# rajan-dubey8/camouflage-multimodal

Hardware: AMD Instinct MI355X
Metric: images/sec fwd+bwd (fusion model train step: fwd + loss + bwd + clip + AdamW) (higher is better)
Workload: dtype bf16; 1 GPU; BASELINE configs[1] on the path that exists (SURVEY 8d): cross-attention fusion model, packed variable-Nr minibatch (Nr ~ real 303..530 histogram, mean 483), Nk=13 real KG rows, train mode dropout 0.3, random-init weights; batch_per_gpu=16, global_batch=16, rg_dim=128, hidden_dim=256, num_heads=8, parallelism=dp1, precision=bf16 MFMA operands, fp32 accumulate/optimizer

## Files before the change

camouflage_multimodal_amd/csrc/common.h:

```cpp
#pragma once
#include <hip/hip_runtime.h>
#include <stdint.h>

#define CAMO_WAVE 64

enum : uint32_t {
  SITE_ATTN_RG2KG = 1, SITE_ATTN_KG2RG = 2, SITE_FFN_RG = 3, SITE_FFN_KG = 4, SITE_FUSE = 5,
  SITE_HEAD0 = 6,
  SITE_LATE0 = 10
};

struct DropCfg {
  uint32_t seed_lo, seed_hi;
  float p;
  float scale;
  uint32_t thr;
};

__host__ __device__ inline DropCfg make_drop(int training, float p, uint64_t seed) {
  DropCfg d;
  d.seed_lo = (uint32_t)(seed & 0xFFFFFFFFull);
  d.seed_hi = (uint32_t)(seed >> 32);
  d.p = (training && p > 0.f) ? p : 0.f;
  d.scale = d.p > 0.f ? 1.0f / (1.0f - d.p) : 1.0f;
  const double t = (double)d.p * 16777216.0;
  unsigned long long t24 = (unsigned long long)t;
  if ((double)t24 < t) ++t24;
  d.thr = t24 >= 16777216ull ? 0xFFFFFFFFu : (uint32_t)(t24 << 8);
  return d;
}

__device__ __forceinline__ uint32_t fmix32(uint32_t x) {
  x ^= x >> 16; x *= 0x85EBCA6Bu; x ^= x >> 13; x *= 0xC2B2AE35u; x ^= x >> 16;
  return x;
}

__device__ __forceinline__ float drop_mult(const DropCfg& d, uint32_t site, uint32_t idx) {
  const uint32_t x = fmix32((idx + (site * 0x85EBCA77u + d.seed_lo)) ^ d.seed_hi);
  return x >= d.thr ? d.scale : 0.0f;
}

extern "C" __device__ int camo_writelane_i32(int, int, int) __asm("llvm.amdgcn.writelane.i32");
#define SET_LANE(v, s, i) (v) = (uint32_t)camo_writelane_i32((int)(s), (i), (int)(v))

__device__ __forceinline__ float wave_sum(float v) {
#pragma unroll
  for (int o = 32; o > 0; o >>= 1) v += __shfl_xor(v, o, 64);
  return v;
}
template <int CTRL, int ROWMASK>
__device__ __forceinline__ float dpp_add(float v) {
  return v + __int_as_float(__builtin_amdgcn_update_dpp(0, __float_as_int(v), CTRL, ROWMASK, 0xf, true));
}
__device__ __forceinline__ float wave_sum_lane63(float v) {
// ... 35 lines not shown
```

camouflage_multimodal_amd/csrc/fused_rows.hip:

```cpp
#include "fused_rows.h"
#include "shadow_inl.h"
#include "gemm.h"
#include "mfma_inl.h"

namespace {

template <int NT, int KS, bool W_IS_A, int DEPTH, bool USE_ROT = true>
struct Stage {
  static constexpr int TOTAL = NT * KS;
  static constexpr int D = DEPTH < TOTAL ? DEPTH : TOTAL;
  static_assert(!USE_ROT || (KS & (KS - 1)) == 0, "rotated k order: power-of-two k steps");
  u32x4 buf[D];
  const u32x4* wp; int rot;
  __device__ __forceinline__ int keff(int ks) const { return USE_ROT ? ((ks + rot) & (KS - 1)) : ks; }
  __device__ __forceinline__ const u32x4* wptr(int i) const { return wp + 64 * (keff(i / NT) * NT + (i % NT)); }
  __device__ __forceinline__ void prefetch(const u32x4* __restrict__ wp_, int rot_) {
    wp = wp_; rot = rot_;
#pragma unroll
    for (int i = 0; i < D; ++i) buf[i] = *wptr(i);
  }
  __device__ __forceinline__ void run(const char* act, f32x16 (&acc)[NT]) {
    run_f([&](int ks) { return *reinterpret_cast<const bf16x8*>(act + 32 * ks); }, acc);
  }
  template <class F>
  __device__ __forceinline__ void run_f(F&& frag, f32x16 (&acc)[NT]) {
    bf16x8 x = frag(keff(0)), xn = x;
#pragma unroll
    for (int i = 0; i < TOTAL; ++i) {
      const int ks = i / NT, t = i % NT;
      const bf16x8 wf = as_frag(buf[i % D]);
      if (i + D < TOTAL) buf[i % D] = *wptr(i + D);
      if (t == 0) {
        x = xn;
        if (ks + 1 < KS) xn = frag(keff(ks + 1));
      }
      if constexpr (W_IS_A) acc[t] = __builtin_amdgcn_mfma_f32_32x32x16_bf16(wf, x, acc[t], 0, 0, 0);
      else                  acc[t] = __builtin_amdgcn_mfma_f32_32x32x16_bf16(x, wf, acc[t], 0, 0, 0);
      __builtin_amdgcn_sched_barrier(0);
    }
  }
};

__device__ __forceinline__ void stamp(unsigned long long* stamps, int k) {
  if (stamps && threadIdx.x == 0) stamps[(size_t)blockIdx.x * 8 + k] = __builtin_amdgcn_s_memrealtime();
}

template <int LOG2C>
__device__ __forceinline__ void copy_out(const char* lds, int pitch, int col_byte0, us16* dst, int ld, size_t row0, int nrows) {
  for (int c = threadIdx.x; c < (32 << LOG2C); c += 256) {
    const int r = c >> LOG2C, k = c & ((1 << LOG2C) - 1);
    if (r < nrows)
      store16_wt(reinterpret_cast<char*>(dst + (row0 + r) * (size_t)ld) + 16 * k, *reinterpret_cast<const u32x4*>(lds + r * pitch + col_byte0 + 16 * k));
  }
}

__global__ __launch_bounds__(256) void shadow_kernel(const ShadowBatch sb, int total_chunks) {
// ... 84 lines not shown
    for (unsigned i = blockIdx.x * 256 + tid; i < n16; i += gridDim.x * 256) z[i] = u32x4{0u, 0u, 0u, 0u};
  }
  stamp(a.stamps, 3);
}

constexpr int PK = 528;
constexpr int PVC = 192;
constexpr int PT = 260;
constexpr int B_VS = 16 * PK;
template <int OCC> struct BackL;
template <> struct BackL<2> { static constexpr int XH = 0, O = 32 * PT * 4, Y = O + 32 * PR, RED = Y + 32 * PR, LDS = RED + 1024; };
template <> struct BackL<3> { static constexpr int Y = 0, XH = 32 * PR, O = 2 * 32 * PR, RED = O + 32 * PR, LDS = RED + 1024; };
constexpr int B_LDS = BackL<2>::LDS;
static_assert(BackL<3>::O >= 4 * 32 * 192 && BackL<3>::O >= 8448 + 9216 && BackL<2>::O >= 4 * 32 * 192, "attention scratch inside region A");

__device__ __forceinline__ void attn_rg_tile(const BackArgs& a, char* smem, char* bufO, int b, size_t row0, int nrows, int w, int lane) {
  const int tid = threadIdx.x, l31 = lane & 31, h = lane >> 5, Nk = a.Nk;
  char* Ks = smem; char* Vs = smem + B_VS;
  for (int c = tid; c < 16 * 64; c += 256) {
    const int j = c >> 6, ch = c & 63;
    u32x4 v = u32x4{0u, 0u, 0u, 0u};
    if (j < Nk) v = *reinterpret_cast<const u32x4*>(a.KV16 + ((size_t)b * Nk + j) * 512 + 8 * ch);
    if (ch < 32) *reinterpret_cast<u32x4*>(Ks + j * PK + 16 * ch) = v;
    else         *reinterpret_cast<u32x4*>(Vs + j * PV + 16 * (ch - 32)) = v;
  }
  const us16* qrow = a.Q16 + (row0 + min(l31, nrows - 1)) * 256 + 64 * w + 8 * h;
  bf16x8 qf[2][2];
#pragma unroll
  for (int hd = 0; hd < 2; ++hd)
#pragma unroll
    for (int s = 0; s < 2; ++s) qf[hd][s] = as_frag(*reinterpret_cast<const u32x4*>(qrow + 32 * hd + 16 * s));
  __syncthreads();
  const bool dodrop = a.drop.p > 0.f;
  const int q4 = (lane >> 2) & 3, p4 = lane & 3, g1 = (lane >> 4) & 1;
#pragma unroll
  for (int hd = 0; hd < 2; ++hd) {
    const int head = 2 * w + hd;
    f32x16 S = zero16();
#pragma unroll
    for (int s = 0; s < 2; ++s) {
      const bf16x8 kf = *reinterpret_cast<const bf16x8*>(Ks + (l31 & 15) * PK + 2 * (32 * head + 16 * s + 8 * h));
      S = __builtin_amdgcn_mfma_f32_32x32x16_bf16(kf, qf[hd][s], S, 0, 0, 0);
    }
    float e[8];
    rg_softmax(S, h, Nk, e);
    const uint32_t ibase = ((uint32_t)(row0 + l31) * 8u + (uint32_t)head) * (uint32_t)Nk;
    if (dodrop) {
#pragma unroll
      for (int i = 0; i < 8; ++i) e[i] *= drop_mult(a.drop, SITE_ATTN_RG2KG, ibase + (uint32_t)acc_row(i, h));
    }
    const bf16x8 pf = as_frag(u32x4{pack2(e[0], e[1]), pack2(e[2], e[3]), pack2(e[4], e[5]), pack2(e[6], e[7])});
    const char* vp = Vs + (4 * h + q4) * PV + 2 * (32 * head + 16 * g1 + 4 * p4);
    const bf16x8 vf = join(lds_tr16(vp), lds_tr16(vp + 8 * PV));
    const f32x16 O = __builtin_amdgcn_mfma_f32_32x32x16_bf16(vf, pf, zero16(), 0, 0, 0);
#pragma unroll
    for (int g = 0; g < 4; ++g)
      *reinterpret_cast<u32x2*>(bufO + l31 * PR + 2 * (32 * head + 8 * g + 4 * h)) =
          u32x2{pack2(O[4 * g], O[4 * g + 1]), pack2(O[4 * g + 2], O[4 * g + 3])};
  }
}

constexpr int SPLIT_ROWS = 64;
constexpr int PART_FLOATS = 16 + 16 + 16 * 32;
static_assert(PART_FLOATS == FUSED_PART_FLOATS, "fused_rows.h");
// ... 13 lines not shown
#pragma unroll
  for (int c = 0; c < 2; ++c) {
    const us16* p = kbase + (size_t)min(r0 + 32 * c + l31, nr - 1) * 512;
#pragma unroll
    for (int hd = 0; hd < 2; ++hd)
#pragma unroll
      for (int s = 0; s < 2; ++s) kf[c][hd][s] = *reinterpret_cast<const u32x4*>(p + 32 * hd + 16 * s);
  }
#pragma unroll
  for (int c = 0; c < 2; ++c)
#pragma unroll
    for (int i = 0; i < 4; ++i) {
      const int id = lane + 64 * i;
      vv[c][i] = *reinterpret_cast<const u32x4*>(vbase + (size_t)min(r0 + 32 * c + (id >> 3), nr - 1) * 512 + 8 * (id & 7));
    }
  f32x16 S[2][2];
  float mx[2] = {-INFINITY, -INFINITY};
#pragma unroll
  for (int c = 0; c < 2; ++c)
#pragma unroll
    for (int hd = 0; hd < 2; ++hd) {
      S[c][hd] = zero16();
#pragma unroll
      for (int s = 0; s < 2; ++s) S[c][hd] = __builtin_amdgcn_mfma_f32_32x32x16_bf16(as_frag(kf[c][hd][s]), qf[hd][s], S[c][hd], 0, 0, 0);
#pragma unroll
      for (int i = 0; i < 16; ++i) mx[hd] = (r0 + 32 * c + acc_row(i, h) < nr) ? fmaxf(mx[hd], S[c][hd][i]) : mx[hd];
    }
  mx[0] = fmaxf(mx[0], __shfl_xor(mx[0], 32, 64));
  mx[1] = fmaxf(mx[1], __shfl_xor(mx[1], 32, 64));
  stamp(a.stamps, 1);
  f32x16 Z[2] = {zero16(), zero16()};
  float L[2] = {0.f, 0.f};
  const bool dodrop = a.drop.p > 0.f;
  const int q4 = (lane >> 2) & 3, p4 = lane & 3, g1 = (lane >> 4) & 1;
#pragma unroll
  for (int c = 0; c < 2; ++c) {
#pragma unroll
    for (int i = 0; i < 4; ++i) { const int id = lane + 64 * i; *reinterpret_cast<u32x4*>(Vt + (id >> 3) * PVC + 16 * (id & 7)) = vv[c][i]; }
#pragma unroll
    for (int hd = 0; hd < 2; ++hd) {
      float e[16];
#pragma unroll
      for (int i = 0; i < 16; ++i) {
        const int row = r0 + 32 * c + acc_row(i, h);
        e[i] = row < nr ? __expf(S[c][hd][i] - mx[hd]) : 0.f;
        L[hd] += e[i];
        if (dodrop) e[i] *= drop_mult(a.drop, SITE_ATTN_KG2RG, ((uint32_t)(rb + row) * 8u + (uint32_t)(2 * w + hd)) * (uint32_t)Nk + (uint32_t)l31);
      }
#pragma unroll
      for (int s = 0; s < 2; ++s) {
        const bf16x8 ef = as_frag(u32x4{pack2(e[8 * s], e[8 * s + 1]), pack2(e[8 * s + 2], e[8 * s + 3]),
                                        pack2(e[8 * s + 4], e[8 * s + 5]), pack2(e[8 * s + 6], e[8 * s + 7])});
        const char* vp = Vt + (16 * s + 4 * h + q4) * PVC + 2 * (32 * hd + 16 * g1 + 4 * p4);
        const bf16x8 vf = join(lds_tr16(vp), lds_tr16(vp + 8 * PVC));
        Z[hd] = __builtin_amdgcn_mfma_f32_32x32x16_bf16(ef, vf, Z[hd], 0, 0, 0);
      }
    }
  }
  L[0] += __shfl_xor(L[0], 32, 64);
  L[1] += __shfl_xor(L[1], 32, 64);
  stamp(a.stamps, 2);
#pragma unroll
// ... 4 lines not shown
      __hip_atomic_store(part + 16 + lane, L[hd], __ATOMIC_RELAXED, __HIP_MEMORY_SCOPE_AGENT);
    }
    float* zt = reinterpret_cast<float*>(Vt);
#pragma unroll
    for (int i = 0; i < 8; ++i) zt[acc_row(i, h) * 32 + l31] = Z[hd][i];
#pragma unroll
    for (int r = 0; r < 2; ++r) {
      const int idx = lane + 64 * r;
      const f32x4 v = *reinterpret_cast<const f32x4*>(zt + 4 * idx);
      float* dst = part + 32 + 4 * idx;
      asm volatile("global_store_dwordx4 %0, %1, off sc1\n\ts_nop 1" ::"v"(dst), "v"(v) : "memory");
    }
  }
}

__device__ __forceinline__ void attn_kg_combine(const BackArgs& a, char* smem, char* bufO, int b, int nsplit) {
  const int tid = threadIdx.x, Nk = a.Nk;
  float* sc = reinterpret_cast<float*>(smem);
  float* invL = sc + nsplit * 128;
  const float* part = a.part + (size_t)a.tile_off[b] * 8 * PART_FLOATS;
  constexpr size_t SS = (size_t)2 * 8 * PART_FLOATS;
  f32x4 zv[4][4];
  auto load_z = [&](int s0) {
#pragma unroll
    for (int k = 0; k < 4; ++k) {
      const float* z = part + (size_t)min(s0 + k, nsplit - 1) * SS + 32;
#pragma unroll
      for (int it = 0; it < 4; ++it) {
        const int idx = tid + 256 * it;
        zv[k][it] = *reinterpret_cast<const f32x4*>(z + (size_t)(idx >> 7) * PART_FLOATS + 4 * (idx & 127));
      }
    }
  };
  load_z(0);
  if (tid < 128) {
    const int hd = tid >> 4, j = tid & 15;
    const float* p0 = part + (size_t)hd * PART_FLOATS + j;
    float M = -INFINITY, L = 0.f;
    if (nsplit <= 16) {
      float mv[16], lv[16];
#pragma unroll
      for (int k = 0; k < 16; ++k) { const size_t o = (size_t)min(k, nsplit - 1) * SS; mv[k] = p0[o]; lv[k] = p0[o + 16]; }
#pragma unroll
      for (int k = 0; k < 16; ++k) M = fmaxf(M, mv[k]);
#pragma unroll
      for (int k = 0; k < 16; ++k)
        if (k < nsplit) { const float e = __expf(mv[k] - M); sc[k * 128 + tid] = e; L = fmaf(lv[k], e, L); }
    } else {
      for (int s0 = 0; s0 < nsplit; s0 += 8) {
        float mv[8];
#pragma unroll
        for (int k = 0; k < 8; ++k) mv[k] = p0[(size_t)min(s0 + k, nsplit - 1) * SS];
#pragma unroll
        for (int k = 0; k < 8; ++k) M = fmaxf(M, mv[k]);
      }
      for (int s0 = 0; s0 < nsplit; s0 += 8) {
        float mv[8], lv[8];
#pragma unroll
        for (int k = 0; k < 8; ++k) { const size_t o = (size_t)min(s0 + k, nsplit - 1) * SS; mv[k] = p0[o]; lv[k] = p0[o + 16]; }
#pragma unroll
        for (int k = 0; k < 8; ++k)
          if (s0 + k < nsplit) { const float e = __expf(mv[k] - M); sc[(s0 + k) * 128 + tid] = e; L = fmaf(lv[k], e, L); }
      }
    }
    invL[tid] = 1.0f / L;
    if ((a.save | a.save_lse2) && a.lse2 && j < Nk) { float* o = a.lse2 + (((size_t)b * 8 + hd) * 16 + j) * 2; o[0] = M; o[1] = L; }
  }
  __syncthreads();
  f32x4 acc[4];
#pragma unroll
  for (int it = 0; it < 4; ++it) acc[it] = f32x4{0.f, 0.f, 0.f, 0.f};
  for (int s0 = 0; s0 < nsplit; s0 += 4) {
    if (s0 > 0) load_z(s0);
#pragma unroll
    for (int k = 0; k < 4; ++k)
      if (s0 + k < nsplit) {
#pragma unroll
        for (int it = 0; it < 4; ++it) acc[it] += zv[k][it] * sc[(s0 + k) * 128 + ((tid + 256 * it) >> 3)];
      }
  }
#pragma unroll
// ... 14 lines not shown
  const int w = __builtin_amdgcn_readfirstlane(tid >> 6);
  const int nkg = a.B * a.max_splits;
  const int vid = (int)blockIdx.x < a.lead_tiles ? nkg + (int)blockIdx.x : ((int)blockIdx.x < a.lead_tiles + nkg ? (int)blockIdx.x - a.lead_tiles : (int)blockIdx.x);
  const bool kg = vid < nkg;
  int rot = ROT ? (int)(blockIdx.x >> 3) : 0;
  using L = BackL<OCC>;
  char* bufO = smem + L::O; char* bufY = smem + L::Y;
  float* red = reinterpret_cast<float*>(smem + L::RED);
  float* tile32 = reinterpret_cast<float*>(smem);
  int b; size_t rowg0; int nrows; float inv_n;
  stamp(a.stamps, 0);
  const BackStream& S = a.s[kg ? 1 : 0];
  Stage<2, 16, true, DEPTH> sto;
  Stage<4, 16, false, DEPTH> stf;
  if (!kg) sto.prefetch(reinterpret_cast<const u32x4*>(S.Wo) + (size_t)w * (16 * 2 * 64) + lane, rot);
  if (kg) {
    b = vid / a.max_splits;
    const int sp = vid - b * a.max_splits;
    if (ROT) rot = b;
    const int nsplit = (a.off[b + 1] - a.off[b] + SPLIT_ROWS - 1) / SPLIT_ROWS;
    if (sp >= nsplit) return;
    attn_kg_split(a, smem, b, sp, w, lane);
    stamp(a.stamps, 4);
    asm volatile("s_waitcnt vmcnt(0)" ::: "memory");
    __syncthreads();
    int* flag = reinterpret_cast<int*>(red);
    if (tid == 0) flag[0] = __hip_atomic_fetch_add(a.tickets + b, 1, __ATOMIC_RELAXED, __HIP_MEMORY_SCOPE_AGENT);
    __syncthreads();
    stamp(a.stamps, 5);
    if (flag[0] != nsplit - 1) return;
    if (tid == 0) {
      __builtin_amdgcn_fence(__ATOMIC_ACQUIRE, "agent");
      asm volatile("s_waitcnt vmcnt(0)" ::: "memory");
    }
    for (int c = tid; c < 32 * PR / 16; c += 256) reinterpret_cast<u32x4*>(bufO)[c] = u32x4{0u, 0u, 0u, 0u};
    __syncthreads();
    sto.prefetch(reinterpret_cast<const u32x4*>(S.Wo) + (size_t)w * (16 * 2 * 64) + lane, rot);
    attn_kg_combine(a, smem, bufO, b, nsplit);
    stamp(a.stamps, 6);
    rowg0 = (size_t)b * a.Nk; nrows = a.Nk; inv_n = 1.0f / (float)a.Nk;
  } else {
    const int4 td = a.tile_desc[vid - nkg];
    if (td.x < 0) return;
    b = td.x; rowg0 = td.y; nrows = td.z; inv_n = __int_as_float(td.w);
    attn_rg_tile(a, smem, bufO, b, rowg0, nrows, w, lane);
  }
  __syncthreads();
  stamp(a.stamps, 1);

  const size_t rrow = rowg0 + min(l31, nrows - 1);
  float u[32];
  float rstd_keep = 0.f;
  {
    f32x16 acc[2] = {zero16(), zero16()};
    sto.run(bufO + l31 * PR + 16 * h, acc);
    stf.prefetch(reinterpret_cast<const u32x4*>(S.W1) + (size_t)w * (16 * 4 * 64) + lane, rot);
    float part = 0.f;
#pragma unroll
    for (int t = 0; t < 2; ++t)
#pragma unroll
// ... 53 lines not shown
      const float tot = ys[0] + __shfl_xor(ys[0], 1, 64);
      if ((l31 & 1) == 0) {
        const int i16 = (l31 >> 1) & 15;
        atomicAdd(S.Ymean + (size_t)b * 256 + 64 * w + 32 * t + 8 * (i16 >> 2) + 4 * h + (i16 & 3), tot * inv_n);
      }
    }
  }
  __syncthreads();
  stamp(a.stamps, 2);
  if constexpr (OCC == 2) {
    float sum = 0.f;
    for (int r = 0; r < nrows; ++r) sum += tile32[r * PT + tid];
    atomicAdd(S.Ymean + (size_t)b * 256 + tid, sum * inv_n);
  }

  {
    f32x16 acc[4] = {zero16(), zero16(), zero16(), zero16()};
    stf.run(bufY + l31 * PR + 16 * h, acc);
    const bool dodrop = a.drop.p > 0.f;
#pragma unroll
    for (int t = 0; t < 4; ++t) {
      const int f = 128 * w + 32 * t + l31;
      const float bias = S.b1[f];
      float colsum = 0.f;
      uint32_t wlo = 0u, whi = 0u;
#pragma unroll
      for (int i = 0; i < 16; ++i) {
        if (8 * (i >> 2) >= nrows) continue;
        const int row = acc_row(i, h);
        float v = fmaxf(acc[t][i] + bias, 0.f);
        if (dodrop) v *= drop_mult(a.drop, S.site_ffn, (uint32_t)(rowg0 + row) * 512u + (uint32_t)f);
        if (row >= nrows) v = 0.f;
        colsum += v;
        if (a.save) {
          const unsigned long long bal = __ballot(v > 0.f);
          SET_LANE(wlo, (uint32_t)bal, i); SET_LANE(whi, (uint32_t)(bal >> 32), i);
        }
      }
      colsum += __shfl_xor(colsum, 32, 64);
      if (h == 0) atomicAdd(S.Hmean + (size_t)b * 512 + f, colsum * inv_n);
      if (a.save && lane < 16) {
        const int ra = acc_row(lane, 0);
        if (ra < nrows) S.mask[(rowg0 + ra) * 16 + 4 * w + t] = wlo;
        if (ra + 4 < nrows) S.mask[(rowg0 + ra + 4) * 16 + 4 * w + t] = whi;
      }
    }
  }
  if (a.save) {
    char* bufXH = smem + L::XH;
    if (w == 0 && h == 0 && l31 < nrows) S.rstd[rowg0 + l31] = rstd_keep;
    __syncthreads();
    if constexpr (OCC == 2) {
#pragma unroll
      for (int t = 0; t < 2; ++t)
#pragma unroll
        for (int g = 0; g < 4; ++g) {
          const float* o = u + 16 * t + 4 * g;
          *reinterpret_cast<u32x2*>(bufXH + l31 * PR + 2 * (64 * w + 32 * t + 8 * g + 4 * h)) = u32x2{pack2(o[0], o[1]), pack2(o[2], o[3])};
        }
      __syncthreads();
    }
    copy_out<5>(bufXH, PR, 0, S.XH16, 256, rowg0, nrows);
// ... 207 lines not shown
    for (int t = 0; t < 2; ++t)
#pragma unroll
      for (int g = 0; g < 4; ++g) {
        const int c0 = 64 * w + 32 * t + 8 * g + 4 * h;
        *reinterpret_cast<float4*>(tile32 + l31 * PT + c0) = make_float4(acc1[t][4 * g], acc1[t][4 * g + 1], acc1[t][4 * g + 2], acc1[t][4 * g + 3]);
      }
    __syncthreads();
    {
      float sum = 0.f;
      for (int r = 0; r < nrows; ++r) sum += tile32[r * PT + tid];
      atomicAdd(S.dbeta + tid, sum);
    }
  }
  stamp(a.stamps, 2);
  f32x16 acc2[2] = {zero16(), zero16()};
  st2.run(bufdU + l31 * PR + 16 * h, acc2);
  copy_out<5>(bufdU, PR, 0, S.dU16, 256, rowg0, nrows);
  if (kg) {
#pragma unroll
    for (int t = 0; t < 2; ++t) {
      float dot = 0.f;
#pragma unroll
      for (int g = 0; g < 4; ++g) {
        const int c0 = 64 * w + 32 * t + 8 * g + 4 * h;
        const u32x2 ov = *reinterpret_cast<const u32x2*>(a.O2_16 + vrow * 256 + c0);
        dot = fmaf(acc2[t][4 * g], bf_lo(ov.x), dot); dot = fmaf(acc2[t][4 * g + 1], bf_hi(ov.x), dot);
        dot = fmaf(acc2[t][4 * g + 2], bf_lo(ov.y), dot); dot = fmaf(acc2[t][4 * g + 3], bf_hi(ov.y), dot);
        if (rok) *reinterpret_cast<u32x2*>(a.dO2_16 + (rowg0 + l31) * 256 + c0) =
            u32x2{pack2(acc2[t][4 * g], acc2[t][4 * g + 1]), pack2(acc2[t][4 * g + 2], acc2[t][4 * g + 3])};
      }
      dot += __shfl_xor(dot, 32, 64);
// ... 2 lines not shown
    stamp(a.stamps, 3);
    return;
  }
  __syncthreads();
#pragma unroll
  for (int i = 0; i < 4; ++i) { const int id = tid + 256 * i; *reinterpret_cast<u32x4*>(bufQ + (id >> 5) * PR + 16 * (id & 31)) = qreg[i]; }
#pragma unroll
  for (int t = 0; t < 2; ++t)
#pragma unroll
    for (int g = 0; g < 4; ++g) {
      const int c0 = 64 * w + 32 * t + 8 * g + 4 * h;
      *reinterpret_cast<u32x2*>(bufdO + l31 * PR + 2 * c0) =
          rok ? u32x2{pack2(acc2[t][4 * g], acc2[t][4 * g + 1]), pack2(acc2[t][4 * g + 2], acc2[t][4 * g + 3])} : u32x2{0u, 0u};
    }
  __syncthreads();
  const bool dodrop = a.drop.p > 0.f;
  const int q4 = (lane >> 2) & 3, p4 = lane & 3, g1 = (lane >> 4) & 1;
#pragma unroll
  for (int t = 0; t < 2; ++t) {
    const int head = 2 * w + t;
    f32x16 Sc = zero16();
#pragma unroll
    for (int s = 0; s < 2; ++s) {
      const bf16x8 kf = *reinterpret_cast<const bf16x8*>(Ks + (l31 & 15) * PK + 2 * (32 * head + 16 * s + 8 * h));
      const bf16x8 qf = *reinterpret_cast<const bf16x8*>(bufQ + l31 * PR + 2 * (32 * head + 16 * s + 8 * h));
      Sc = __builtin_amdgcn_mfma_f32_32x32x16_bf16(kf, qf, Sc, 0, 0, 0);
    }
    float pr[8], mm[8];
    rg_softmax(Sc, h, a.Nk, pr);
    const uint32_t ibase = ((uint32_t)(rowg0 + l31) * 8u + (uint32_t)head) * (uint32_t)a.Nk;
#pragma unroll
    for (int i = 0; i < 8; ++i) mm[i] = dodrop ? drop_mult(a.drop, SITE_ATTN_RG2KG, ibase + (uint32_t)acc_row(i, h)) : 1.0f;
    f32x16 dP = zero16();
#pragma unroll
    for (int s = 0; s < 2; ++s) {
      const char* vp = Vs + (l31 & 15) * PK + 2 * (32 * head + 16 * s + 4 * h);
      const u32x2 v0 = *reinterpret_cast<const u32x2*>(vp), v1 = *reinterpret_cast<const u32x2*>(vp + 16);
      const bf16x8 vf = as_frag(u32x4{v0.x, v0.y, v1.x, v1.y});
      const bf16x8 of = as_frag(u32x4{pack2(acc2[t][8 * s], acc2[t][8 * s + 1]), pack2(acc2[t][8 * s + 2], acc2[t][8 * s + 3]),
                                      pack2(acc2[t][8 * s + 4], acc2[t][8 * s + 5]), pack2(acc2[t][8 * s + 6], acc2[t][8 * s + 7])});
      dP = __builtin_amdgcn_mfma_f32_32x32x16_bf16(vf, of, dP, 0, 0, 0);
    }
    float ds[8], pd[8], delta = 0.f;
#pragma unroll
    for (int i = 0; i < 8; ++i) { ds[i] = dP[i] * mm[i]; delta = fmaf(pr[i], ds[i], delta); pd[i] = pr[i] * mm[i]; }
    delta += __shfl_xor(delta, 32, 64);
#pragma unroll
// ... 104 lines not shown
          __hip_atomic_store(dst + 1, acc[t][4 * g + 1] + bf_hi(uv.x), __ATOMIC_RELAXED, __HIP_MEMORY_SCOPE_AGENT);
          __hip_atomic_store(dst + 2, acc[t][4 * g + 2] + bf_lo(uv.y), __ATOMIC_RELAXED, __HIP_MEMORY_SCOPE_AGENT);
          __hip_atomic_store(dst + 3, acc[t][4 * g + 3] + bf_hi(uv.y), __ATOMIC_RELAXED, __HIP_MEMORY_SCOPE_AGENT);
        }
    }
  } else {
  const int4 td = a.tile_desc[(int)blockIdx.x - a.B];
  if (td.x < 0) return;
  b = td.x;
  const size_t rowg0 = td.y;
  const int nrows = td.z;
  const bool rok = l31 < nrows;
  const size_t vrow = rowg0 + min(l31, nrows - 1);
  Stage<2, 48, true, DEPTH, false> sr;
  sr.prefetch(reinterpret_cast<const u32x4*>(a.WcRgT) + (size_t)w * (48 * 2 * 64) + lane, 0);
  for (int c = tid; c < 16 * 32; c += 256) {
    const int j = c >> 5, ch = c & 31;
    u32x4 q = u32x4{0u, 0u, 0u, 0u}, o = q;
    if (j < Nk) {
      q = *reinterpret_cast<const u32x4*>(a.Q2_16 + ((size_t)b * Nk + j) * 256 + 8 * ch);
      o = *reinterpret_cast<const u32x4*>(a.dO2_16 + ((size_t)b * Nk + j) * 256 + 8 * ch);
    }
    *reinterpret_cast<u32x4*>(Q2s + j * PK + 16 * ch) = q;
    *reinterpret_cast<u32x4*>(dO2s + j * PK + 16 * ch) = o;
  }
  if (tid < 128) {
    const int j = tid & 15;
    const size_t o = (size_t)b * 128 + tid;
    const bool ok = j < Nk;
    tabs[tid] = ok ? a.lse2[2 * o] : 0.f;
    tabs[128 + tid] = ok ? 1.0f / a.lse2[2 * o + 1] : 0.f;
    tabs[256 + tid] = ok ? a.delta2[o] : 0.f;
  }
  u32x4 dqreg[4];
#pragma unroll
  for (int i = 0; i < 4; ++i) {
    const int id = tid + 256 * i;
    const size_t r = rowg0 + min(id >> 5, nrows - 1);
    *reinterpret_cast<u32x4*>(bufT + (id >> 5) * PQ + 16 * (id & 31)) = *reinterpret_cast<const u32x4*>(a.KV2_16 + r * 512 + 8 * (id & 31));
    dqreg[i] = *reinterpret_cast<const u32x4*>(a.dQKV16 + r * 768 + 8 * (id & 31));
  }
  bf16x8 kf[2][2], vf[2][2];
  {
    const us16* kp = a.KV2_16 + vrow * 512 + 64 * w + 8 * h;
#pragma unroll
    for (int t = 0; t < 2; ++t)
#pragma unroll
      for (int s = 0; s < 2; ++s) {
        kf[t][s] = as_frag(*reinterpret_cast<const u32x4*>(kp + 32 * t + 16 * s));
        vf[t][s] = as_frag(*reinterpret_cast<const u32x4*>(kp + 256 + 32 * t + 16 * s));
      }
  }
  __syncthreads();
  const bool dodrop = a.drop.p > 0.f;
  const int q4 = (lane >> 2) & 3, p4 = lane & 3, g1 = (lane >> 4) & 1;
#pragma unroll
  for (int t = 0; t < 2; ++t) {
    const int head = 2 * w + t;
    f32x16 S2 = zero16(), dP = zero16();
#pragma unroll
    for (int s = 0; s < 2; ++s) {
      const int co = (l31 & 15) * PK + 2 * (32 * head + 16 * s + 8 * h);
      S2 = __builtin_amdgcn_mfma_f32_32x32x16_bf16(*reinterpret_cast<const bf16x8*>(Q2s + co), kf[t][s], S2, 0, 0, 0);
      dP = __builtin_amdgcn_mfma_f32_32x32x16_bf16(*reinterpret_cast<const bf16x8*>(dO2s + co), vf[t][s], dP, 0, 0, 0);
    }
    float ds[8], pd[8];
#pragma unroll
    for (int i = 0; i < 8; ++i) {
      const int j = acc_row(i, h);
      const float p = (j < Nk && rok) ? __expf(S2[i] - tabs[head * 16 + j]) * tabs[128 + head * 16 + j] : 0.f;
      const float mm = dodrop ? drop_mult(a.drop, SITE_ATTN_KG2RG, ((uint32_t)(rowg0 + l31) * 8u + (uint32_t)head) * (uint32_t)Nk + (uint32_t)j) : 1.0f;
      ds[i] = p * (dP[i] * mm - tabs[256 + head * 16 + j]);
      pd[i] = p * mm;
    }
    const u32x4 dsf = u32x4{pack2(ds[0], ds[1]), pack2(ds[2], ds[3]), pack2(ds[4], ds[5]), pack2(ds[6], ds[7])};
    const u32x4 pdf = u32x4{pack2(pd[0], pd[1]), pack2(pd[2], pd[3]), pack2(pd[4], pd[5]), pack2(pd[6], pd[7])};
    const int tro = (4 * h + q4) * PK + 2 * (32 * head + 16 * g1 + 4 * p4);
    const f32x16 dv = __builtin_amdgcn_mfma_f32_32x32x16_bf16(join(lds_tr16(dO2s + tro), lds_tr16(dO2s + tro + 8 * PK)), as_frag(pdf), zero16(), 0, 0, 0);
    const f32x16 dk = __builtin_amdgcn_mfma_f32_32x32x16_bf16(join(lds_tr16(Q2s + tro), lds_tr16(Q2s + tro + 8 * PK)), as_frag(dsf), zero16(), 0, 0, 0);
#pragma unroll
    for (int g = 0; g < 4; ++g) {
      const int c = 32 * head + 8 * g + 4 * h;
      *reinterpret_cast<u32x2*>(bufT + l31 * PQ + 2 * (256 + c)) = u32x2{pack2(dk[4 * g], dk[4 * g + 1]), pack2(dk[4 * g + 2], dk[4 * g + 3])};
      *reinterpret_cast<u32x2*>(bufT + l31 * PQ + 2 * (512 + c)) = u32x2{pack2(dv[4 * g], dv[4 * g + 1]), pack2(dv[4 * g + 2], dv[4 * g + 3])};
    }
    char* im = imgs + head * 1024;
// ... 391 lines not shown
```

camouflage_multimodal_amd/csrc/misc.hip:

```cpp
#include "misc.h"
#include "gemm.h"


namespace {

__global__ __launch_bounds__(256) void batchdesc_kernel(const int* __restrict__ offs, int* __restrict__ row_sample, float* __restrict__ inv_nr,
                                                        int* __restrict__ tile_off, int4* __restrict__ tile_desc, int B, int ntile_max) {
  __shared__ int part[256];
  __shared__ int total_s;
  const int t = threadIdx.x, per = (B + 255) / 256, b0 = min(B, t * per), b1 = min(B, b0 + per);
  const int T = offs[B];
  int s = 0;
  for (int b = b0; b < b1; ++b) s += (offs[b + 1] - offs[b] + 31) >> 5;
  {
    const int lane = t & 63, w = t >> 6;
    int incl = s;
#pragma unroll
    for (int o = 1; o < 64; o <<= 1) { const int v = __shfl_up(incl, o, 64); if (lane >= o) incl += v; }
    if (lane == 63) part[w] = incl;
    __syncthreads();
    const int w0 = part[0], w1 = part[1], w2 = part[2], w3 = part[3];
    __syncthreads();
    const int base = w == 0 ? 0 : (w == 1 ? w0 : (w == 2 ? w0 + w1 : w0 + w1 + w2));
    part[t] = base + incl - s;
// ... 703 lines not shown
  if (tid < 256) reinterpret_cast<float4*>(WfL)[tid] = wfl;
  __syncthreads();
  tstamp(a.stamps, 2);
  if (active) {
    float w8[8];
#pragma unroll
    for (int c = 0; c < 8; ++c) w8[c] = wB[t * 8 + c];
#pragma unroll
    for (int j = 0; j < 4; ++j) {
      const float4 ca = reinterpret_cast<const float4*>(combS)[(b0 + j) * 2], cb = reinterpret_cast<const float4*>(combS)[(b0 + j) * 2 + 1];
      const float acc = bias2 + w8[0] * ca.x + w8[1] * ca.y + w8[2] * ca.z + w8[3] * ca.w + w8[4] * cb.x + w8[5] * cb.y + w8[6] * cb.z + w8[7] * cb.w;
      if (b0 + j < B) atomicAdd(gF1sum + (b0 + j) * 256 + t, acc);
    }
  }
  tstamp(a.stamps, 3);
  tail_arrive_wait(cnt + 0, gaveup, &s_timed_out, a.debug_skip == (int)blockIdx.x + 1);
  tstamp(a.stamps, 4);
  {
    const float4 v4 = tid < B * 64 ? reinterpret_cast<const float4*>(gF1sum)[tid] : z4;
    if (tid < B4 * 64) {
      float v[4] = {fmaxf(v4.x, 0.f), fmaxf(v4.y, 0.f), fmaxf(v4.z, 0.f), fmaxf(v4.w, 0.f)};
      if (dodrop) {
#pragma unroll
        for (int e = 0; e < 4; ++e) v[e] *= drop_mult(a.drop, SITE_FUSE, (uint32_t)(sb * 256 + 4 * tid + e));
      }
      reinterpret_cast<float4*>(F1)[tid] = make_float4(v[0], v[1], v[2], v[3]);
      if (wg && g == 0 && tid < B * 64) reinterpret_cast<float4*>(gF1_out)[tid] = make_float4(v[0], v[1], v[2], v[3]);
    }
  }
  __syncthreads();
  tstamp(a.stamps, 5);
  if (active) {
    float acc[4] = {0.f, 0.f, 0.f, 0.f};
#pragma unroll
    for (int i = 0; i < 4; ++i)
#pragma unroll
      for (int j = 0; j < 4; ++j) acc[j] = fmaf(WfL[wv * 256 + lane + 64 * i], F1[(b0 + j) * 256 + lane + 64 * i], acc[j]);
    wave_sum4(acc);
    if (lane == 63) {
// ... 6 lines not shown
  }
  __syncthreads();
  tstamp(a.stamps, 6);
  if (active) {
    const float4 wa0 = reinterpret_cast<const float4*>(wA)[t], wa1 = reinterpret_cast<const float4*>(wA)[t + 256];
#pragma unroll
    for (int j = 0; j < 4; ++j) {
      const float4 f = reinterpret_cast<const float4*>(fusedS)[b0 + j];
      if (b0 + j < B) {
        atomicAdd(ghidsum + (b0 + j) * 512 + t, bias4a + wa0.x * f.x + wa0.y * f.y + wa0.z * f.z + wa0.w * f.w);
        atomicAdd(ghidsum + (b0 + j) * 512 + t + 256, bias4b + wa1.x * f.x + wa1.y * f.y + wa1.z * f.z + wa1.w * f.w);
      }
    }
  }
  tstamp(a.stamps, 7);
  tail_arrive_wait(cnt + 1, gaveup, &s_timed_out);
  tstamp(a.stamps, 8);
  {
    float4 v4[2];
#pragma unroll
    for (int it = 0; it < 2; ++it) { const int i = tid + TF_THREADS * it; v4[it] = i < B * 128 ? reinterpret_cast<const float4*>(ghidsum)[i] : z4; }
#pragma unroll
    for (int it = 0; it < 2; ++it) {
      const int i = tid + TF_THREADS * it;
      if (i < B4 * 128) {
        float v[4] = {fmaxf(v4[it].x, 0.f), fmaxf(v4[it].y, 0.f), fmaxf(v4[it].z, 0.f), fmaxf(v4[it].w, 0.f)};
        if (dodrop) {
          const int b = sb + (i >> 7), m = (4 * i) & 511;
#pragma unroll
          for (int e = 0; e < 4; ++e) v[e] *= drop_mult(a.drop, SITE_HEAD0 + (uint32_t)(m >> 7), (uint32_t)(b * 128 + (m & 127) + e));
        }
        reinterpret_cast<float4*>(R2)[i] = make_float4(v[0], v[1], v[2], v[3]);
      }
    }
  }
  if (tid < TF_MAXB * TF_MAXW) dpre[tid] = 0.f;
  __syncthreads();
  tstamp(a.stamps, 9);
#pragma unroll 1
  for (int p = tid >> 2; p < B * Wd; p += TF_THREADS / 4) {
    const int kq = tid & 3;
    const int b = p / Wd, o = p - b * Wd;
    const int x = o < C ? 0 : (o < 2 * C ? 1 : (o == 2 * C ? 2 : 3));
    const float* wr = w3s + o * 129 + 4 * kq;
    const float* hr = R2 + b * 512 + x * 128 + 4 * kq;
// ... 645 lines not shown
```

Baseline: 97420 images/s.

## Precompute dropout keep masks early to overlap hashing with loads and MFMA

Dropout hash evaluation moves out of the softmax and FFN epilogue inner loops. Keep bits are now computed ahead of time into packed bitmasks: while global loads of K/V/Q tiles are in flight, interleaved between MFMA steps through a side callback, or before the grid-wide tail barriers in the head kernel. LDS stores are also deferred until after the hash work so memory latency overlaps ALU. The FFN epilogue is specialised at compile time on drop and save and splits full from partial row groups. This raises register pressure and code size, and relies on sched_barrier and asm pinning to hold the intended placement.

```diff
diff --git a/camouflage_multimodal_amd/csrc/common.h b/camouflage_multimodal_amd/csrc/common.h
--- a/camouflage_multimodal_amd/csrc/common.h
+++ b/camouflage_multimodal_amd/csrc/common.h
@@ -35,9 +35,11 @@
   return x;
 }
 
+__device__ __forceinline__ bool drop_keep(const DropCfg& d, uint32_t site, uint32_t idx) {
+  return fmix32((idx + (site * 0x85EBCA77u + d.seed_lo)) ^ d.seed_hi) >= d.thr;
+}
 __device__ __forceinline__ float drop_mult(const DropCfg& d, uint32_t site, uint32_t idx) {
-  const uint32_t x = fmix32((idx + (site * 0x85EBCA77u + d.seed_lo)) ^ d.seed_hi);
-  return x >= d.thr ? d.scale : 0.0f;
+  return drop_keep(d, site, idx) ? d.scale : 0.0f;
 }
 
 extern "C" __device__ int camo_writelane_i32(int, int, int) __asm("llvm.amdgcn.writelane.i32");
diff --git a/camouflage_multimodal_amd/csrc/fused_rows.hip b/camouflage_multimodal_amd/csrc/fused_rows.hip
--- a/camouflage_multimodal_amd/csrc/fused_rows.hip
+++ b/camouflage_multimodal_amd/csrc/fused_rows.hip
@@ -1,3 +1,4 @@
+#include <type_traits>
 #include "fused_rows.h"
 #include "shadow_inl.h"
 #include "gemm.h"
@@ -19,11 +20,13 @@
 #pragma unroll
     for (int i = 0; i < D; ++i) buf[i] = *wptr(i);
   }
-  __device__ __forceinline__ void run(const char* act, f32x16 (&acc)[NT]) {
-    run_f([&](int ks) { return *reinterpret_cast<const bf16x8*>(act + 32 * ks); }, acc);
-  }
-  template <class F>
-  __device__ __forceinline__ void run_f(F&& frag, f32x16 (&acc)[NT]) {
+  struct NoSide { __device__ __forceinline__ void operator()(int) const {} };
+  template <class G = NoSide>
+  __device__ __forceinline__ void run(const char* act, f32x16 (&acc)[NT], G&& side = G()) {
+    run_f([&](int ks) { return *reinterpret_cast<const bf16x8*>(act + 32 * ks); }, acc, side);
+  }
+  template <class F, class G = NoSide>
+  __device__ __forceinline__ void run_f(F&& frag, f32x16 (&acc)[NT], G&& side = G()) {
     bf16x8 x = frag(keff(0)), xn = x;
 #pragma unroll
     for (int i = 0; i < TOTAL; ++i) {
@@ -36,10 +39,13 @@
       }
       if constexpr (W_IS_A) acc[t] = __builtin_amdgcn_mfma_f32_32x32x16_bf16(wf, x, acc[t], 0, 0, 0);
       else                  acc[t] = __builtin_amdgcn_mfma_f32_32x32x16_bf16(x, wf, acc[t], 0, 0, 0);
+      side(i);
       __builtin_amdgcn_sched_barrier(0);
     }
   }
 };
+
+#define PIN_HERE(v) asm volatile("" : "+v"(v))
 
 __device__ __forceinline__ void stamp(unsigned long long* stamps, int k) {
   if (stamps && threadIdx.x == 0) stamps[(size_t)blockIdx.x * 8 + k] = __builtin_amdgcn_s_memrealtime();
@@ -154,15 +160,16 @@
 constexpr int B_LDS = BackL<2>::LDS;
 static_assert(BackL<3>::O >= 4 * 32 * 192 && BackL<3>::O >= 8448 + 9216 && BackL<2>::O >= 4 * 32 * 192, "attention scratch inside region A");
 
-__device__ __forceinline__ void attn_rg_tile(const BackArgs& a, char* smem, char* bufO, int b, size_t row0, int nrows, int w, int lane) {
+template <class G>
+__device__ __forceinline__ void attn_rg_tile(const BackArgs& a, char* smem, char* bufO, int b, size_t row0, int nrows, int w, int lane, G&& ahead) {
   const int tid = threadIdx.x, l31 = lane & 31, h = lane >> 5, Nk = a.Nk;
   char* Ks = smem; char* Vs = smem + B_VS;
-  for (int c = tid; c < 16 * 64; c += 256) {
-    const int j = c >> 6, ch = c & 63;
-    u32x4 v = u32x4{0u, 0u, 0u, 0u};
-    if (j < Nk) v = *reinterpret_cast<const u32x4*>(a.KV16 + ((size_t)b * Nk + j) * 512 + 8 * ch);
-    if (ch < 32) *reinterpret_cast<u32x4*>(Ks + j * PK + 16 * ch) = v;
-    else         *reinterpret_cast<u32x4*>(Vs + j * PV + 16 * (ch - 32)) = v;
+  u32x4 kv[4];
+#pragma unroll
+  for (int i = 0; i < 4; ++i) {
+    const int c = tid + 256 * i, j = c >> 6, ch = c & 63;
+    kv[i] = u32x4{0u, 0u, 0u, 0u};
+    if (j < Nk) kv[i] = *reinterpret_cast<const u32x4*>(a.KV16 + ((size_t)b * Nk + j) * 512 + 8 * ch);
   }
   const us16* qrow = a.Q16 + (row0 + min(l31, nrows - 1)) * 256 + 64 * w + 8 * h;
   bf16x8 qf[2][2];
@@ -170,8 +177,27 @@
   for (int hd = 0; hd < 2; ++hd)
 #pragma unroll
     for (int s = 0; s < 2; ++s) qf[hd][s] = as_frag(*reinterpret_cast<const u32x4*>(qrow + 32 * hd + 16 * s));
-  __syncthreads();
   const bool dodrop = a.drop.p > 0.f;
+  uint32_t keep = 0u;
+  __builtin_amdgcn_sched_barrier(0);
+  if (dodrop) {
+#pragma unroll
+    for (int hd = 0; hd < 2; ++hd) {
+      const uint32_t ibase = ((uint32_t)(row0 + l31) * 8u + (uint32_t)(2 * w + hd)) * (uint32_t)Nk;
+#pragma unroll
+      for (int i = 0; i < 8; ++i) keep |= drop_keep(a.drop, SITE_ATTN_RG2KG, ibase + (uint32_t)acc_row(i, h)) ? 1u << (8 * hd + i) : 0u;
+    }
+    PIN_HERE(keep);
+  }
+  ahead();
+  __builtin_amdgcn_sched_barrier(0);
+#pragma unroll
+  for (int i = 0; i < 4; ++i) {
+    const int c = tid + 256 * i, j = c >> 6, ch = c & 63;
+    if (ch < 32) *reinterpret_cast<u32x4*>(Ks + j * PK + 16 * ch) = kv[i];
+    else         *reinterpret_cast<u32x4*>(Vs + j * PV + 16 * (ch - 32)) = kv[i];
+  }
+  __syncthreads();
   const int q4 = (lane >> 2) & 3, p4 = lane & 3, g1 = (lane >> 4) & 1;
 #pragma unroll
   for (int hd = 0; hd < 2; ++hd) {
@@ -184,10 +210,9 @@
     }
     float e[8];
     rg_softmax(S, h, Nk, e);
-    const uint32_t ibase = ((uint32_t)(row0 + l31) * 8u + (uint32_t)head) * (uint32_t)Nk;
     if (dodrop) {
 #pragma unroll
-      for (int i = 0; i < 8; ++i) e[i] *= drop_mult(a.drop, SITE_ATTN_RG2KG, ibase + (uint32_t)acc_row(i, h));
+      for (int i = 0; i < 8; ++i) e[i] = (keep >> (8 * hd + i)) & 1u ? e[i] * a.drop.scale : 0.0f;
     }
     const bf16x8 pf = as_frag(u32x4{pack2(e[0], e[1]), pack2(e[2], e[3]), pack2(e[4], e[5]), pack2(e[6], e[7])});
     const char* vp = Vs + (4 * h + q4) * PV + 2 * (32 * head + 16 * g1 + 4 * p4);
@@ -231,6 +256,22 @@
       const int id = lane + 64 * i;
       vv[c][i] = *reinterpret_cast<const u32x4*>(vbase + (size_t)min(r0 + 32 * c + (id >> 3), nr - 1) * 512 + 8 * (id & 7));
     }
+  const bool dodrop = a.drop.p > 0.f;
+  uint32_t keep[2] = {0u, 0u};
+  __builtin_amdgcn_sched_barrier(0);
+  if (dodrop) {
+#pragma unroll
+    for (int c = 0; c < 2; ++c)
+#pragma unroll
+      for (int hd = 0; hd < 2; ++hd)
+#pragma unroll
+        for (int i = 0; i < 16; ++i) {
+          const int row = r0 + 32 * c + acc_row(i, h);
+          keep[c] |= drop_keep(a.drop, SITE_ATTN_KG2RG, ((uint32_t)(rb + row) * 8u + (uint32_t)(2 * w + hd)) * (uint32_t)Nk + (uint32_t)l31) ? 1u << (16 * hd + i) : 0u;
+        }
+    PIN_HERE(keep[0]); PIN_HERE(keep[1]);
+  }
+  __builtin_amdgcn_sched_barrier(0);
   f32x16 S[2][2];
   float mx[2] = {-INFINITY, -INFINITY};
 #pragma unroll
@@ -248,8 +289,9 @@
   stamp(a.stamps, 1);
   f32x16 Z[2] = {zero16(), zero16()};
   float L[2] = {0.f, 0.f};
-  const bool dodrop = a.drop.p > 0.f;
   const int q4 = (lane >> 2) & 3, p4 = lane & 3, g1 = (lane >> 4) & 1;
+  const float dscale = dodrop ? a.drop.scale : 1.0f;
+  if (!dodrop) keep[0] = keep[1] = 0xFFFFFFFFu;
 #pragma unroll
   for (int c = 0; c < 2; ++c) {
 #pragma unroll
@@ -260,9 +302,10 @@
 #pragma unroll
       for (int i = 0; i < 16; ++i) {
         const int row = r0 + 32 * c + acc_row(i, h);
-        e[i] = row < nr ? __expf(S[c][hd][i] - mx[hd]) : 0.f;
-        L[hd] += e[i];
-        if (dodrop) e[i] *= drop_mult(a.drop, SITE_ATTN_KG2RG, ((uint32_t)(rb + row) * 8u + (uint32_t)(2 * w + hd)) * (uint32_t)Nk + (uint32_t)l31);
+        const float ex = __expf(S[c][hd][i] - mx[hd]);
+        const float ev = row < nr ? ex : 0.f;
+        L[hd] += ev;
+        e[i] = (keep[c] >> (16 * hd + i)) & 1u ? ev * dscale : 0.0f;
       }
 #pragma unroll
       for (int s = 0; s < 2; ++s) {
@@ -297,7 +340,8 @@
   }
 }
 
-__device__ __forceinline__ void attn_kg_combine(const BackArgs& a, char* smem, char* bufO, int b, int nsplit) {
+template <class G>
+__device__ __forceinline__ void attn_kg_combine(const BackArgs& a, char* smem, char* bufO, int b, int nsplit, G&& ahead) {
   const int tid = threadIdx.x, Nk = a.Nk;
   float* sc = reinterpret_cast<float*>(smem);
   float* invL = sc + nsplit * 128;
@@ -324,12 +368,16 @@
       float mv[16], lv[16];
 #pragma unroll
       for (int k = 0; k < 16; ++k) { const size_t o = (size_t)min(k, nsplit - 1) * SS; mv[k] = p0[o]; lv[k] = p0[o + 16]; }
+      __builtin_amdgcn_sched_barrier(0);
+      ahead();
+      __builtin_amdgcn_sched_barrier(0);
 #pragma unroll
       for (int k = 0; k < 16; ++k) M = fmaxf(M, mv[k]);
 #pragma unroll
       for (int k = 0; k < 16; ++k)
         if (k < nsplit) { const float e = __expf(mv[k] - M); sc[k * 128 + tid] = e; L = fmaf(lv[k], e, L); }
     } else {
+      ahead();
       for (int s0 = 0; s0 < nsplit; s0 += 8) {
         float mv[8];
 #pragma unroll
@@ -348,6 +396,10 @@
     }
     invL[tid] = 1.0f / L;
     if ((a.save | a.save_lse2) && a.lse2 && j < Nk) { float* o = a.lse2 + (((size_t)b * 8 + hd) * 16 + j) * 2; o[0] = M; o[1] = L; }
+  } else {
+    __builtin_amdgcn_sched_barrier(0);
+    ahead();
+    __builtin_amdgcn_sched_barrier(0);
   }
   __syncthreads();
   f32x4 acc[4];
@@ -392,6 +444,23 @@
   Stage<2, 16, true, DEPTH> sto;
   Stage<4, 16, false, DEPTH> stf;
   if (!kg) sto.prefetch(reinterpret_cast<const u32x4*>(S.Wo) + (size_t)w * (16 * 2 * 64) + lane, rot);
+  const bool dodrop = a.drop.p > 0.f;
+  constexpr bool AHEAD = OCC == 2;
+  uint32_t keep[2] = {0u, 0u};
+  auto draw_ffn = [&](size_t rowg0_, int nrows_) __attribute__((always_inline)) {
+    if (!(AHEAD && dodrop)) return;
+    const uint32_t lane0 = ((uint32_t)(rowg0_ + 4 * h) * 512u + (uint32_t)(128 * w + l31)) + (S.site_ffn * 0x85EBCA77u + a.drop.seed_lo);
+#pragma unroll
+    for (int g = 0; g < 4; ++g) {
+      if (8 * g >= nrows_) break;
+#pragma unroll
+      for (int t = 0; t < 4; ++t)
+#pragma unroll
+        for (int i = 4 * g; i < 4 * g + 4; ++i)
+          keep[t >> 1] |= fmix32((lane0 + (uint32_t)(512 * acc_row(i, 0) + 32 * t)) ^ a.drop.seed_hi) >= a.drop.thr ? 1u << (16 * (t & 1) + i) : 0u;
+      PIN_HERE(keep[0]); PIN_HERE(keep[1]);
+    }
+  };
   if (kg) {
     b = vid / a.max_splits;
     const int sp = vid - b * a.max_splits;
@@ -414,14 +483,14 @@
     for (int c = tid; c < 32 * PR / 16; c += 256) reinterpret_cast<u32x4*>(bufO)[c] = u32x4{0u, 0u, 0u, 0u};
     __syncthreads();
     sto.prefetch(reinterpret_cast<const u32x4*>(S.Wo) + (size_t)w * (16 * 2 * 64) + lane, rot);
-    attn_kg_combine(a, smem, bufO, b, nsplit);
+    rowg0 = (size_t)b * a.Nk; nrows = a.Nk; inv_n = 1.0f / (float)a.Nk;
+    attn_kg_combine(a, smem, bufO, b, nsplit, [&]() __attribute__((always_inline)) { draw_ffn(rowg0, nrows); });
     stamp(a.stamps, 6);
-    rowg0 = (size_t)b * a.Nk; nrows = a.Nk; inv_n = 1.0f / (float)a.Nk;
   } else {
     const int4 td = a.tile_desc[vid - nkg];
     if (td.x < 0) return;
     b = td.x; rowg0 = td.y; nrows = td.z; inv_n = __int_as_float(td.w);
-    attn_rg_tile(a, smem, bufO, b, rowg0, nrows, w, lane);
+    attn_rg_tile(a, smem, bufO, b, rowg0, nrows, w, lane, [&]() __attribute__((always_inline)) { draw_ffn(rowg0, nrows); });
   }
   __syncthreads();
   stamp(a.stamps, 1);
@@ -505,38 +574,46 @@
     atomicAdd(S.Ymean + (size_t)b * 256 + tid, sum * inv_n);
   }
 
-  {
-    f32x16 acc[4] = {zero16(), zero16(), zero16(), zero16()};
-    stf.run(bufY + l31 * PR + 16 * h, acc);
-    const bool dodrop = a.drop.p > 0.f;
+  f32x16 acc[4] = {zero16(), zero16(), zero16(), zero16()};
+  stf.run(bufY + l31 * PR + 16 * h, acc);
+  auto ffn_epilogue = [&](auto drop_c, auto save_c) __attribute__((always_inline)) {
+    constexpr bool DROP = decltype(drop_c)::value, SAVE = decltype(save_c)::value;
 #pragma unroll
     for (int t = 0; t < 4; ++t) {
       const int f = 128 * w + 32 * t + l31;
       const float bias = S.b1[f];
       float colsum = 0.f;
       uint32_t wlo = 0u, whi = 0u;
-#pragma unroll
-      for (int i = 0; i < 16; ++i) {
-        if (8 * (i >> 2) >= nrows) continue;
-        const int row = acc_row(i, h);
-        float v = fmaxf(acc[t][i] + bias, 0.f);
-        if (dodrop) v *= drop_mult(a.drop, S.site_ffn, (uint32_t)(rowg0 + row) * 512u + (uint32_t)f);
-        if (row >= nrows) v = 0.f;
-        colsum += v;
-        if (a.save) {
-          const unsigned long long bal = __ballot(v > 0.f);
-          SET_LANE(wlo, (uint32_t)bal, i); SET_LANE(whi, (uint32_t)(bal >> 32), i);
+      auto group = [&](int g, auto part_c) __attribute__((always_inline)) {
+#pragma unroll
+        for (int i = 4 * g; i < 4 * g + 4; ++i) {
+          float v = fmaxf(acc[t][i] + bias, 0.f);
+          if constexpr (DROP && AHEAD) v = (keep[t >> 1] >> (16 * (t & 1) + i)) & 1u ? v * a.drop.scale : 0.0f;
+          if constexpr (DROP && !AHEAD) v *= drop_mult(a.drop, S.site_ffn, (uint32_t)(rowg0 + acc_row(i, h)) * 512u + (uint32_t)f);
+          if constexpr (decltype(part_c)::value) v = acc_row(i, h) < nrows ? v : 0.f;
+          colsum += v;
+          if constexpr (SAVE) {
+            const unsigned long long bal = __ballot(v > 0.f);
+            SET_LANE(wlo, (uint32_t)bal, i); SET_LANE(whi, (uint32_t)(bal >> 32), i);
+          }
         }
+      };
+#pragma unroll
+      for (int g = 0; g < 4; ++g) {
+        if (8 * g + 8 <= nrows) group(g, std::false_type());
+        else if (8 * g < nrows) group(g, std::true_type());
       }
       colsum += __shfl_xor(colsum, 32, 64);
       if (h == 0) atomicAdd(S.Hmean + (size_t)b * 512 + f, colsum * inv_n);
-      if (a.save && lane < 16) {
+      if (SAVE && lane < 16) {
         const int ra = acc_row(lane, 0);
         if (ra < nrows) S.mask[(rowg0 + ra) * 16 + 4 * w + t] = wlo;
         if (ra + 4 < nrows) S.mask[(rowg0 + ra + 4) * 16 + 4 * w + t] = whi;
       }
     }
-  }
+  };
+  if (dodrop) { if (a.save) ffn_epilogue(std::true_type(), std::true_type()); else ffn_epilogue(std::true_type(), std::false_type()); }
+  else        { if (a.save) ffn_epilogue(std::false_type(), std::true_type()); else ffn_epilogue(std::false_type(), std::false_type()); }
   if (a.save) {
     char* bufXH = smem + L::XH;
     if (w == 0 && h == 0 && l31 < nrows) S.rstd[rowg0 + l31] = rstd_keep;
@@ -774,7 +851,16 @@
   }
   stamp(a.stamps, 2);
   f32x16 acc2[2] = {zero16(), zero16()};
-  st2.run(bufdU + l31 * PR + 16 * h, acc2);
+  const bool dodrop = a.drop.p > 0.f;
+  uint32_t keep = 0u;
+  if (dodrop && !kg) {
+    const uint32_t i0 = (uint32_t)(rowg0 + l31) * 8u + (uint32_t)(2 * w);
+    st2.run(bufdU + l31 * PR + 16 * h, acc2, [&](int s) __attribute__((always_inline)) {
+      if (s < 16) { keep |= drop_keep(a.drop, SITE_ATTN_RG2KG, (i0 + (uint32_t)(s >> 3)) * (uint32_t)a.Nk + (uint32_t)acc_row(s & 7, h)) ? 1u << s : 0u; PIN_HERE(keep); }
+    });
+  } else {
+    st2.run(bufdU + l31 * PR + 16 * h, acc2);
+  }
   copy_out<5>(bufdU, PR, 0, S.dU16, 256, rowg0, nrows);
   if (kg) {
 #pragma unroll
@@ -807,7 +893,6 @@
           rok ? u32x2{pack2(acc2[t][4 * g], acc2[t][4 * g + 1]), pack2(acc2[t][4 * g + 2], acc2[t][4 * g + 3])} : u32x2{0u, 0u};
     }
   __syncthreads();
-  const bool dodrop = a.drop.p > 0.f;
   const int q4 = (lane >> 2) & 3, p4 = lane & 3, g1 = (lane >> 4) & 1;
 #pragma unroll
   for (int t = 0; t < 2; ++t) {
@@ -821,9 +906,8 @@
     }
     float pr[8], mm[8];
     rg_softmax(Sc, h, a.Nk, pr);
-    const uint32_t ibase = ((uint32_t)(rowg0 + l31) * 8u + (uint32_t)head) * (uint32_t)a.Nk;
-#pragma unroll
-    for (int i = 0; i < 8; ++i) mm[i] = dodrop ? drop_mult(a.drop, SITE_ATTN_RG2KG, ibase + (uint32_t)acc_row(i, h)) : 1.0f;
+#pragma unroll
+    for (int i = 0; i < 8; ++i) mm[i] = dodrop ? ((keep >> (8 * t + i)) & 1u ? a.drop.scale : 0.0f) : 1.0f;
     f32x16 dP = zero16();
 #pragma unroll
     for (int s = 0; s < 2; ++s) {
@@ -958,30 +1042,27 @@
   const size_t vrow = rowg0 + min(l31, nrows - 1);
   Stage<2, 48, true, DEPTH, false> sr;
   sr.prefetch(reinterpret_cast<const u32x4*>(a.WcRgT) + (size_t)w * (48 * 2 * 64) + lane, 0);
-  for (int c = tid; c < 16 * 32; c += 256) {
-    const int j = c >> 5, ch = c & 31;
-    u32x4 q = u32x4{0u, 0u, 0u, 0u}, o = q;
+  u32x4 qv[2], ov[2];
+#pragma unroll
+  for (int it = 0; it < 2; ++it) {
+    const int c = tid + 256 * it, j = c >> 5, ch = c & 31;
+    qv[it] = u32x4{0u, 0u, 0u, 0u}; ov[it] = qv[it];
     if (j < Nk) {
-      q = *reinterpret_cast<const u32x4*>(a.Q2_16 + ((size_t)b * Nk + j) * 256 + 8 * ch);
-      o = *reinterpret_cast<const u32x4*>(a.dO2_16 + ((size_t)b * Nk + j) * 256 + 8 * ch);
-    }
-    *reinterpret_cast<u32x4*>(Q2s + j * PK + 16 * ch) = q;
-    *reinterpret_cast<u32x4*>(dO2s + j * PK + 16 * ch) = o;
-  }
-  if (tid < 128) {
-    const int j = tid & 15;
+      qv[it] = *reinterpret_cast<const u32x4*>(a.Q2_16 + ((size_t)b * Nk + j) * 256 + 8 * ch);
+      ov[it] = *reinterpret_cast<const u32x4*>(a.dO2_16 + ((size_t)b * Nk + j) * 256 + 8 * ch);
+    }
+  }
+  float tv[3] = {0.f, 0.f, 0.f};
+  if (tid < 128 && (tid & 15) < Nk) {
     const size_t o = (size_t)b * 128 + tid;
-    const bool ok = j < Nk;
-    tabs[tid] = ok ? a.lse2[2 * o] : 0.f;
-    tabs[128 + tid] = ok ? 1.0f / a.lse2[2 * o + 1] : 0.f;
-    tabs[256 + tid] = ok ? a.delta2[o] : 0.f;
-  }
-  u32x4 dqreg[4];
+    tv[0] = a.lse2[2 * o]; tv[1] = a.lse2[2 * o + 1]; tv[2] = a.delta2[o];
+  }
+  u32x4 ktile[4], dqreg[4];
 #pragma unroll
   for (int i = 0; i < 4; ++i) {
     const int id = tid + 256 * i;
     const size_t r = rowg0 + min(id >> 5, nrows - 1);
-    *reinterpret_cast<u32x4*>(bufT + (id >> 5) * PQ + 16 * (id & 31)) = *reinterpret_cast<const u32x4*>(a.KV2_16 + r * 512 + 8 * (id & 31));
+    ktile[i] = *reinterpret_cast<const u32x4*>(a.KV2_16 + r * 512 + 8 * (id & 31));
     dqreg[i] = *reinterpret_cast<const u32x4*>(a.dQKV16 + r * 768 + 8 * (id & 31));
   }
   bf16x8 kf[2][2], vf[2][2];
@@ -995,8 +1076,33 @@
         vf[t][s] = as_frag(*reinterpret_cast<const u32x4*>(kp + 256 + 32 * t + 16 * s));
       }
   }
-  __syncthreads();
+  __builtin_amdgcn_sched_barrier(0);
   const bool dodrop = a.drop.p > 0.f;
+  uint32_t keep = 0u;
+  if (dodrop) {
+#pragma unroll
+    for (int t = 0; t < 2; ++t)
+#pragma unroll
+      for (int i = 0; i < 8; ++i)
+        keep |= drop_keep(a.drop, SITE_ATTN_KG2RG, ((uint32_t)(rowg0 + l31) * 8u + (uint32_t)(2 * w + t)) * (uint32_t)Nk + (uint32_t)acc_row(i, h)) ? 1u << (8 * t + i) : 0u;
+    PIN_HERE(keep);
+  }
+  __builtin_amdgcn_sched_barrier(0);
+#pragma unroll
+  for (int it = 0; it < 2; ++it) {
+    const int c = tid + 256 * it, j = c >> 5, ch = c & 31;
+    *reinterpret_cast<u32x4*>(Q2s + j * PK + 16 * ch) = qv[it];
+    *reinterpret_cast<u32x4*>(dO2s + j * PK + 16 * ch) = ov[it];
+  }
+  if (tid < 128) {
+    const bool ok = (tid & 15) < Nk;
+    tabs[tid] = tv[0];
+    tabs[128 + tid] = ok ? 1.0f / tv[1] : 0.f;
+    tabs[256 + tid] = tv[2];
+  }
+#pragma unroll
+  for (int i = 0; i < 4; ++i) { const int id = tid + 256 * i; *reinterpret_cast<u32x4*>(bufT + (id >> 5) * PQ + 16 * (id & 31)) = ktile[i]; }
+  __syncthreads();
   const int q4 = (lane >> 2) & 3, p4 = lane & 3, g1 = (lane >> 4) & 1;
 #pragma unroll
   for (int t = 0; t < 2; ++t) {
@@ -1013,7 +1119,7 @@
     for (int i = 0; i < 8; ++i) {
       const int j = acc_row(i, h);
       const float p = (j < Nk && rok) ? __expf(S2[i] - tabs[head * 16 + j]) * tabs[128 + head * 16 + j] : 0.f;
-      const float mm = dodrop ? drop_mult(a.drop, SITE_ATTN_KG2RG, ((uint32_t)(rowg0 + l31) * 8u + (uint32_t)head) * (uint32_t)Nk + (uint32_t)j) : 1.0f;
+      const float mm = dodrop ? ((keep >> (8 * t + i)) & 1u ? a.drop.scale : 0.0f) : 1.0f;
       ds[i] = p * (dP[i] * mm - tabs[256 + head * 16 + j]);
       pd[i] = p * mm;
     }
diff --git a/camouflage_multimodal_amd/csrc/misc.hip b/camouflage_multimodal_amd/csrc/misc.hip
--- a/camouflage_multimodal_amd/csrc/misc.hip
+++ b/camouflage_multimodal_amd/csrc/misc.hip
@@ -741,6 +741,11 @@
     }
   }
   tstamp(a.stamps, 3);
+  float dm1[4] = {1.f, 1.f, 1.f, 1.f}, dm2[2][4] = {{1.f, 1.f, 1.f, 1.f}, {1.f, 1.f, 1.f, 1.f}};
+  if (dodrop && tid < B4 * 64) {
+#pragma unroll
+    for (int e = 0; e < 4; ++e) dm1[e] = drop_mult(a.drop, SITE_FUSE, (uint32_t)(sb * 256 + 4 * tid + e));
+  }
   tail_arrive_wait(cnt + 0, gaveup, &s_timed_out, a.debug_skip == (int)blockIdx.x + 1);
   tstamp(a.stamps, 4);
   {
@@ -749,7 +754,7 @@
       float v[4] = {fmaxf(v4.x, 0.f), fmaxf(v4.y, 0.f), fmaxf(v4.z, 0.f), fmaxf(v4.w, 0.f)};
       if (dodrop) {
 #pragma unroll
-        for (int e = 0; e < 4; ++e) v[e] *= drop_mult(a.drop, SITE_FUSE, (uint32_t)(sb * 256 + 4 * tid + e));
+        for (int e = 0; e < 4; ++e) v[e] *= dm1[e];
       }
       reinterpret_cast<float4*>(F1)[tid] = make_float4(v[0], v[1], v[2], v[3]);
       if (wg && g == 0 && tid < B * 64) reinterpret_cast<float4*>(gF1_out)[tid] = make_float4(v[0], v[1], v[2], v[3]);
@@ -786,6 +791,17 @@
     }
   }
   tstamp(a.stamps, 7);
+  if (dodrop) {
+#pragma unroll
+    for (int it = 0; it < 2; ++it) {
+      const int i = tid + TF_THREADS * it;
+      if (i < B4 * 128) {
+        const int b = sb + (i >> 7), m = (4 * i) & 511;
+#pragma unroll
+        for (int e = 0; e < 4; ++e) dm2[it][e] = drop_mult(a.drop, SITE_HEAD0 + (uint32_t)(m >> 7), (uint32_t)(b * 128 + (m & 127) + e));
+      }
+    }
+  }
   tail_arrive_wait(cnt + 1, gaveup, &s_timed_out);
   tstamp(a.stamps, 8);
   {
@@ -798,9 +814,8 @@
       if (i < B4 * 128) {
         float v[4] = {fmaxf(v4[it].x, 0.f), fmaxf(v4[it].y, 0.f), fmaxf(v4[it].z, 0.f), fmaxf(v4[it].w, 0.f)};
         if (dodrop) {
-          const int b = sb + (i >> 7), m = (4 * i) & 511;
-#pragma unroll
-          for (int e = 0; e < 4; ++e) v[e] *= drop_mult(a.drop, SITE_HEAD0 + (uint32_t)(m >> 7), (uint32_t)(b * 128 + (m & 127) + e));
+#pragma unroll
+          for (int e = 0; e < 4; ++e) v[e] *= dm2[it][e];
         }
         reinterpret_cast<float4*>(R2)[i] = make_float4(v[0], v[1], v[2], v[3]);
       }
```

Measured after the change: 98230 images/s, median of 6. Within noise of the previous version (+0.8%).
